# thomascbrs/mpc-tsid

Hardware: AMD Instinct MI355X
Metric: QP instances/s (12-state, N=16) at 1/2/4/8 MI355X; max |f - f_osqp| (higher is better)
Workload: dtype f64

## Files before the change

mpc-tsid_amd/csrc/mpcq_engine.hip:

```cpp
#include <math.h>

#include <type_traits>
#include <utility>

#include "mpcq_internal.h"

namespace mpcq {
namespace {

typedef __attribute__((address_space(3))) const double lds_cd;
typedef __attribute__((address_space(3))) double lds_d;
typedef double dbl2 __attribute__((ext_vector_type(2)));
typedef __attribute__((address_space(3))) const dbl2 lds_cd2;
typedef __attribute__((address_space(1))) const double g_cd;
typedef __attribute__((address_space(1))) double g_d;
typedef __attribute__((address_space(1))) const dbl2 g_cd2;

constexpr double kInf = 1e30;
constexpr double kMinScaling = 1e-4, kMaxScaling = 1e4;
constexpr double kRhoMin = 1e-6, kRhoMax = 1e6, kRhoEq = 1e3, kRhoTol = 1e-4;
constexpr double kDivTol = 1e-30;

enum : unsigned { RC_LOOSE = 0, RC_INEQ = 1, RC_EQ = 2 };

#if defined(MPCQ_STAMPS) && defined(MPCQ_STAMPS_LEAN)
#define STAMP_DECL uint64_t st_acc[16] = {}; uint64_t st_last = __builtin_amdgcn_s_memtime();
#define STAMP(i) do { if constexpr ((i) == 1 || (i) == 2 || (i) == 3 || (i) == 7 || (i) == 10 || (i) == 11 || (i) == 12) { \
    const uint64_t nw_ = __builtin_amdgcn_s_memtime(); st_acc[i] += nw_ - st_last; st_last = nw_; } } while (0)
#elif defined(MPCQ_STAMPS)
#define STAMP_DECL uint64_t st_acc[16] = {}; uint64_t st_last = __builtin_amdgcn_s_memtime();
#define STAMP(i) do { if (threadIdx.x == kStampT) { const uint64_t nw_ = __builtin_amdgcn_s_memtime(); st_acc[i] += nw_ - st_last; st_last = nw_; } } while (0)
#else
#define STAMP_DECL
#define STAMP(i) do {} while (0)
#endif

template <int N>
__device__ __forceinline__ int XO(int k, int i) {
  return (k < N - 1) ? 30 * k + (i < 6 ? 2 * i : 12 + 3 * (i - 6)) : 30 * (N - 1) + i;
}
template <int N>
__device__ __forceinline__ int FO(int k, int f, int c) {
  return 30 * N - 18 + 96 * k + 24 * f + 7 * c;
}
__host__ __device__ constexpr int LN(int psi) { return 4 * (psi / 3) + psi % 3; }

template <int N>
__host__ __device__ constexpr int SIG(int k) { return k <= N / 2 ? k : N + N / 2 - k; }
template <int N>
__host__ __device__ constexpr int SIGX(int q) { return q <= N / 2 ? q : N + N / 2 + 1 - q; }

template <int N>
constexpr int kRows = (N + 3) & ~3;
template <int N>
constexpr bool kSlice = slice_supported(N);


__device__ __forceinline__ void wave_sync() {
  __builtin_amdgcn_fence(__ATOMIC_RELEASE, "wavefront");
  __builtin_amdgcn_wave_barrier();
  asm volatile("" ::: "memory");
  __builtin_amdgcn_fence(__ATOMIC_ACQUIRE, "wavefront");
}
__device__ __forceinline__ void sync_all() { __syncthreads(); }

template <int CTRL>
__device__ __forceinline__ double dppd(double v) {
  return __longlong_as_double(__builtin_amdgcn_mov_dpp(__double_as_longlong(v), CTRL, 0xF, 0xF, false));
}
template <int J>
__device__ __forceinline__ double rbc(double v) { return dppd<0x150 + J>(v); }
template <int J>
__device__ __forceinline__ double qbc(double v) { return dppd<85 * J>(v); }
template <int J0, int J1, int J2, int J3>
__device__ __forceinline__ double qperm(double v) { return dppd<J0 + 4 * J1 + 16 * J2 + 64 * J3>(v); }

#define MPCQ_HV(i) "+v"(a[i])
#define MPCQ_HV4(i) MPCQ_HV(i), MPCQ_HV(i + 1), MPCQ_HV(i + 2), MPCQ_HV(i + 3)
template <int n>
__device__ __forceinline__ void hold_all(double (&a)[n]) {
  static_assert((n >= 1 && n <= 8) || n == 15 || n == 21, "hold_all: spell this count out");
  if constexpr (n == 1) asm volatile("" : MPCQ_HV(0));
  if constexpr (n == 2) asm volatile("" : MPCQ_HV(0), MPCQ_HV(1));
  if constexpr (n == 3) asm volatile("" : MPCQ_HV(0), MPCQ_HV(1), MPCQ_HV(2));
  if constexpr (n == 4) asm volatile("" : MPCQ_HV4(0));
  if constexpr (n == 5) asm volatile("" : MPCQ_HV4(0), MPCQ_HV(4));
  if constexpr (n == 6) asm volatile("" : MPCQ_HV4(0), MPCQ_HV(4), MPCQ_HV(5));
  if constexpr (n == 7) asm volatile("" : MPCQ_HV4(0), MPCQ_HV(4), MPCQ_HV(5), MPCQ_HV(6));
  if constexpr (n == 8) asm volatile("" : MPCQ_HV4(0), MPCQ_HV4(4));
  if constexpr (n == 15) asm volatile("" : MPCQ_HV4(0), MPCQ_HV4(4), MPCQ_HV4(8), MPCQ_HV(12), MPCQ_HV(13), MPCQ_HV(14));
  if constexpr (n == 21) asm volatile("" : MPCQ_HV4(0), MPCQ_HV4(4), MPCQ_HV4(8), MPCQ_HV4(12), MPCQ_HV4(16), MPCQ_HV(20));
}
#undef MPCQ_HV4
#undef MPCQ_HV

__device__ __forceinline__ double bdot12(const double (&g)[12], double v, double i0) {
  double a0 = i0;
  asm volatile("s_nop 1\n\t"
      "v_fmac_f64_dpp %0, %1, %2 row_newbcast:0 row_mask:0xf bank_mask:0xf\n\t"
      "v_fmac_f64_dpp %0, %1, %3 row_newbcast:1 row_mask:0xf bank_mask:0xf\n\t"
      "v_fmac_f64_dpp %0, %1, %4 row_newbcast:2 row_mask:0xf bank_mask:0xf\n\t"
      "v_fmac_f64_dpp %0, %1, %5 row_newbcast:3 row_mask:0xf bank_mask:0xf\n\t"
      "v_fmac_f64_dpp %0, %1, %6 row_newbcast:4 row_mask:0xf bank_mask:0xf\n\t"
      "v_fmac_f64_dpp %0, %1, %7 row_newbcast:5 row_mask:0xf bank_mask:0xf\n\t"
      "v_fmac_f64_dpp %0, %1, %8 row_newbcast:6 row_mask:0xf bank_mask:0xf\n\t"
      "v_fmac_f64_dpp %0, %1, %9 row_newbcast:7 row_mask:0xf bank_mask:0xf\n\t"
      "v_fmac_f64_dpp %0, %1, %10 row_newbcast:8 row_mask:0xf bank_mask:0xf\n\t"
      "v_fmac_f64_dpp %0, %1, %11 row_newbcast:9 row_mask:0xf bank_mask:0xf\n\t"
      "v_fmac_f64_dpp %0, %1, %12 row_newbcast:10 row_mask:0xf bank_mask:0xf\n\t"
      "v_fmac_f64_dpp %0, %1, %13 row_newbcast:11 row_mask:0xf bank_mask:0xf"
      : "+v"(a0)
      : "v"(v), "v"(g[0]), "v"(g[1]), "v"(g[2]), "v"(g[3]), "v"(g[4]), "v"(g[5]), "v"(g[6]), "v"(g[7]),
        "v"(g[8]), "v"(g[9]), "v"(g[10]), "v"(g[11]));
  return a0;
}
__device__ __forceinline__ double bdot_ln12(const double (&g)[12], double v, double i0) {
  double a0 = i0;
  asm("s_nop 1\n\t"
      "v_fmac_f64_dpp %0, %1, %2 row_newbcast:0 row_mask:0xf bank_mask:0xf\n\t"
      "v_fmac_f64_dpp %0, %1, %3 row_newbcast:1 row_mask:0xf bank_mask:0xf\n\t"
      "v_fmac_f64_dpp %0, %1, %4 row_newbcast:2 row_mask:0xf bank_mask:0xf\n\t"
      "v_fmac_f64_dpp %0, %1, %5 row_newbcast:4 row_mask:0xf bank_mask:0xf\n\t"
      "v_fmac_f64_dpp %0, %1, %6 row_newbcast:5 row_mask:0xf bank_mask:0xf\n\t"
      "v_fmac_f64_dpp %0, %1, %7 row_newbcast:6 row_mask:0xf bank_mask:0xf\n\t"
      "v_fmac_f64_dpp %0, %1, %8 row_newbcast:8 row_mask:0xf bank_mask:0xf\n\t"
      "v_fmac_f64_dpp %0, %1, %9 row_newbcast:9 row_mask:0xf bank_mask:0xf\n\t"
      "v_fmac_f64_dpp %0, %1, %10 row_newbcast:10 row_mask:0xf bank_mask:0xf\n\t"
      "v_fmac_f64_dpp %0, %1, %11 row_newbcast:12 row_mask:0xf bank_mask:0xf\n\t"
      "v_fmac_f64_dpp %0, %1, %12 row_newbcast:13 row_mask:0xf bank_mask:0xf\n\t"
      "v_fmac_f64_dpp %0, %1, %13 row_newbcast:14 row_mask:0xf bank_mask:0xf"
      : "+v"(a0)
      : "v"(v), "v"(g[0]), "v"(g[1]), "v"(g[2]), "v"(g[3]), "v"(g[4]), "v"(g[5]), "v"(g[6]), "v"(g[7]),
        "v"(g[8]), "v"(g[9]), "v"(g[10]), "v"(g[11]));
  return a0;
// ... 760 lines not shown
        return cl ? 0.0 : kInf;
      } else {
        return hi_g[j];
      }
    };

    using pdbl = __attribute__((address_space(5))) double;
    enum { ZC_LO = 0, ZC_HI = 3, ZC_RR = 6, ZC_RI = 9, ZC_COUNT = 12 };
    double zc_mem_[kZcMem<N> ? ZC_COUNT : 1];
    auto zc_ptr = [&]() __attribute__((always_inline)) -> pdbl* {
      pdbl* q = (pdbl*)&zc_mem_[0];
      asm volatile("" : "+v"(q));
      return q;
    };
    auto zc_store = [&]() __attribute__((always_inline)) {
      if constexpr (kZcMem<N>) {
        pdbl* const q = zc_ptr();
#pragma unroll
        for (int j = 0; j < 3; ++j) {
          q[ZC_LO + j] = lo_of(j);
          q[ZC_HI + j] = hi_of(j);
          q[ZC_RR + j] = rr[j];
          q[ZC_RI + j] = ri[j];
        }
      }
    };

    auto row_A = [&](double vf, double vX, double (&out)[3]) __attribute__((always_inline)) {
      double fall[12];
      gather12(vf, fall);
      const double* xp = sh.u.it.xs[k];
      const double hd = Hd(k, ph), h6 = H6(k, ph);
      const double xa = xp[ph], xb = xp[ph < 6 ? ph + 6 : ph];
      double dyn = Xd(k, ph) * vX;
      const double d1 = dyn + hd * xa;
      const double d2 = d1 + h6 * xb;
      dyn = k >= 1 ? (ph < 6 ? d2 : d1) : dyn;
      double bcf[12];
#pragma unroll
      for (int psi = 0; psi < 12; ++psi) bcf[psi] = Bc(k, ph, psi / 3, psi % 3);
      const double bf = dot12(bcf, fall);
      dyn = ph >= 6 ? dyn + bf : dyn;
      const double g0 = qbc<0>(vf), g1 = qbc<1>(vf), g2 = qbc<2>(vf);
      const double swg = Ab[fo + 4] * vf;
      out[0] = cl ? dyn : fric_row(3, g0, g1, g2);
      out[1] = cl ? swg : fric_row(4, g0, g1, g2);
      out[2] = cl ? fric_row(c, g0, g1, g2) : 0.0;
    };
    auto Pbf = [&]() __attribute__((always_inline)) { return cscale * (Df * P0f * Df); };
    auto PbX = [&]() __attribute__((always_inline)) { return cscale * (DX * P0X * DX); };

    auto rdy = [&](int kk, int i) __attribute__((always_inline)) { return GHr[GS * kk + 108 + i]; };
    auto Qv = [&](int kk, int j1, int j2) __attribute__((always_inline)) { return GHr[GS * kk + 6 * j1 + j2]; };
    auto Ctop = [&](int kk, int i, double& ca, double (&c6)[6]) __attribute__((always_inline)) {
      const int iq = i >= 6 ? i - 6 : 0;
      const double ri = rdy(kk, i), xi = Xd(kk, i), hi = Hd(kk, i), h6 = H6(kk, i < 6 ? i : 0);
      const double dv = ri * xi * hi, tv = ri * xi * h6;
      ca = i < 6 ? dv : 0.0;
#pragma unroll
      for (int j = 0; j < 6; ++j) {
        const double sc = xi * Qv(kk, iq, j) * Hd(kk, 6 + j);
        const double vv = (6 + j == i ? dv : 0.0) - sc;
        c6[j] = i < 6 ? (j == i ? tv : 0.0) : vv;
      }
    };
    auto Cbot = [&](int kk, int i, double& ca, double (&c6)[6]) __attribute__((always_inline)) {
      const int ip = i >= 6 ? i - 6 : 0;
      const double hi = Hd(kk, i);
      const double dv = rdy(kk, i) * Xd(kk, i) * hi;
      const double tv = rdy(kk, ip) * Xd(kk, ip) * H6(kk, ip);
      ca = i < 6 ? dv : tv;
#pragma unroll
      for (int j = 0; j < 6; ++j) {
        const double sc = Xd(kk, 6 + j) * Qv(kk, j, ip) * hi;
        const double vv = (6 + j == i ? dv : 0.0) - sc;
        c6[j] = i >= 6 ? vv : 0.0;
      }
    };
    auto Drow = [&](int kk, int i, double diag0, double (&Dr)[12]) __attribute__((always_inline)) {
      const bool nx = kk < N - 1;
      const int k1 = nx ? kk + 1 : kk;
      const int i6 = i < 6 ? i : i - 6, iq = i >= 6 ? i - 6 : 0;
      const double xi = Xd(kk, i), ri0 = rdy(kk, i);
      const double hi1 = Hd(k1, i), ri1 = rdy(k1, i);
      const double h6p = H6(k1, i6), rp1 = rdy(k1, i6), hp1 = Hd(k1, i6);
      double dg = diag0 + ri0 * xi * xi;
      const double dn = ri1 * hi1 * hi1 + (i >= 6 ? rp1 * h6p * h6p : 0.0);
      dg = nx ? dg + dn : dg;
      const double cross = nx ? (i < 6 ? ri1 * hi1 * h6p : rp1 * hp1 * h6p) : 0.0;
      const int partner = i < 6 ? i + 6 : i - 6;
#pragma unroll
      for (int ci = 0; ci < 12; ++ci) {
        double v = (ci == i) ? dg : 0.0;
        v = (ci == partner) ? cross : v;
        if (ci >= 6) {
          const double s0 = xi * Qv(kk, iq, ci - 6) * Xd(kk, ci);
          const double s1 = hi1 * Qv(k1, iq, ci - 6) * Hd(k1, ci);
          v = i >= 6 ? v - (nx ? s0 + s1 : s0) : v;
        }
        Dr[ci] = v;
      }
    };

      auto ph_sweep_lag = [&]() __attribute__((always_inline)) {
          const int half = (t >> 5) & 1;
#ifndef MPCQ_REP_SWEEP
#define MPCQ_REP_SWEEP 1
#endif
#pragma nounroll
          for (int rep_ = 0; rep_ < MPCQ_REP_SWEEP; ++rep_) {
          double xp = 0.0;
          using swp = lds_cd;
          using swp2 = lds_cd2;
          swp* const GHs = GHr;
          swp* const Mb = half == 0 ? GHs + (GS * (cr == 0 ? 0 : MID) + (cr == 0 ? 0 : kSlotPad<N>) + RS * rr_)
                                    : (swp*)&sh.Sm[0][0] + (GS * (cr == 0 ? -2 : MID - 1) + (cr == 0 ? 0 : kSlotPad<N>) + RS * rr_);
          double g[12];
          auto row12 = [&](swp* q) __attribute__((always_inline)) {
#pragma unroll
            for (int i = 0; i < 6; ++i) {
              const dbl2 v = ((swp2*)q)[i];
              g[2 * i] = v.x;
              g[2 * i + 1] = v.y;
            }
          };
          auto rowp = [&](int j) __attribute__((always_inline)) -> swp* {
            if (j >= 2 && j <= BOT) return Mb + GS * j;
            const int jj = half == 0 ? (cr == 0 ? j : (j < BOT ? j : BOT))
                                     : (cr == 0 ? (j > 2 ? j : 2) : (j < BOT + 1 ? j : BOT + 1));
            return Mb + GS * jj;
          };
          STAMP(15);
          if (t < 64) row12(rowp(1));
          sync_all();
          STAMP(3);
          lds_cd* const Ob = GHr + (GS * (cr == 0 ? 1 : N - MID) + (cr == 0 ? 0 : kSlotPad<N>) + rr_);
          if (t < 64) {
            __builtin_amdgcn_s_setprio(3);
            lds_cd* const Bb = (lds_cd*)&sh.u.it.bo[0][0] + (12 * (cr == 0 ? 0 : MID + 1) + rr_);
            lds_cd* const Bm = (lds_cd*)&sh.u.it.bo[0][0] + (12 * MID + rr_);
            auto rhs = [&](int j) __attribute__((always_inline)) -> lds_cd* {
              return (j >= BOT && cr != 0) ? Bm : Bb + 12 * j;
            };
            lds_d* const sink = (lds_d*)&sh.red[0] + (t & 31);
            lds_d* const Yb = (half == 1 && s < 12) ? (lds_d*)&sh.u.it.yv[0][0] + (12 * (cr == 0 ? -2 : MID - 1) + rr_)
                                                    : sink;
            lds_d* const Ym = ((N & 1) || cr == 0) ? Yb + 12 * (MID + 1) : sink;
            lds_d* const Pm = (half == 0 && cr == 0 && s < 12)
                                  ? (lds_d*)&sh.u.it.xs[0][0] + (12 * SIGX<N>(MID + 1) + rr_) : Ym;
            const double m0 = half == 0 ? 1.0 : 0.0;
// ... 30 lines not shown
              if (j >= 2 && j <= MID) {
                Yb[12 * j] = acc;
              } else if (j == MID + 1) {
                *Pm = acc;
              }
              if (j <= MID) {
                const bool adv = j <= BOT || cr == 0;
                src = keep_lo_take_lo(adv ? acc : src, src);
                asm volatile("" : "+v"(src));
              } else {
                xp = acc;
              }
            }
            STAMP(6);
          }
          if (t < 64) {
            lds_cd* const Wb = (lds_cd*)&sh.u.it.yv[0][0] + (12 * (cr == 0 ? 0 : N - MID) + rr_);
            lds_d* const sinkO = (lds_d*)&sh.red[0] + (t & 31);
            lds_d* const Xb = (half == 0 && s < 12) ? (lds_d*)&sh.u.it.xs[0][0] + (12 * (cr == 0 ? 1 : N - MID) + rr_)
                                                    : sinkO;
            wave_sync();
            double bq = Wb[12 * (MID - 1)];
#pragma unroll
            for (int j = 1; j <= MID; ++j) {
              asm volatile("" : : : "memory");
              double gc[12];
#pragma unroll
              for (int i = 0; i < 12; ++i) gc[i] = g[i];
              const double bc = bq;
              if (j < MID) {
#pragma unroll
                for (int i = 0; i < 12; ++i) g[i] = Ob[RS * i + GS * (MID - j - 1)];
                if (j + 1 <= BOT) bq = Wb[12 * (MID - j - 1)];
                else bq = Wb[12 * (MID - (cr == 0 ? j + 1 : BOT))];
              }
              asm volatile("" : : : "memory");
              const double acc = bdot12(gc, xp, bc);
              if (j < MID) {
                xp = acc;
                Xb[12 * (MID - j)] = acc;
              } else if constexpr (N & 1) {
                *Xb = acc;
              } else {
                *(cr == 0 ? Xb : sinkO) = acc;
              }
            }
            __builtin_amdgcn_s_setprio(0);
          }
          wave_sync();
          }
      };
    auto factor = [&](double sigma, const double* pr) __attribute__((always_inline)) -> bool {
      bool ok = true;
      launder();
      auto rho_of = [&](int j) __attribute__((always_inline)) -> double {
        return pr ? pr[j] : rho_of_cls(j);
      };
      double* gk = gh0 + GS * k;
      if (cl) gk[108 + ph] = rho_of(0);
      sync_all();
      {
        double rd6[6];
#pragma unroll
        for (int j = 0; j < 6; ++j) rd6[j] = gk[114 + j];
        double rfr[5];
        {
          const double r0 = rho_of(0), r1 = rho_of(1), r2 = rho_of(2);
          rfr[0] = qbc<0>(r2); rfr[1] = qbc<1>(r2); rfr[2] = qbc<2>(r2);
          rfr[3] = qbc<3>(r0); rfr[4] = qbc<3>(r1);
        }
        const double Bo0 = Ab[fo], Bo1 = Ab[fo + 1], Bo2 = Ab[fo + 2], Bo3 = Ab[fo + 3];
        const double sw = Ab[fo + 4];
        const double rsw = rho_of(1);
        double own_fr[5];
#pragma unroll
        for (int t_ = 0; t_ < 5; ++t_) own_fr[t_] = rfr[t_] * Frc(k, f, t_, cc);
        const double dgf = Pbf() + sigma + rsw * sw * sw;
#pragma unroll
        for (int psi = 0; psi < 12; ++psi) {
          const int fp = psi / 3, cp = psi % 3;
          double v = (cp == cc) ? rd6[cp] * Bo0 * Ab[FO<N>(k, fp, cp)] : 0.0;
          v += rd6[3] * Bo1 * Ab[FO<N>(k, fp, cp) + 1];
          v += rd6[4] * Bo2 * Ab[FO<N>(k, fp, cp) + 2];
          v += rd6[5] * Bo3 * Ab[FO<N>(k, fp, cp) + 3];
          if (psi == ph) v += dgf;
          if (fp == f) {
            double fr = 0.0;
#pragma unroll
            for (int t_ = 0; t_ < 5; ++t_) fr += own_fr[t_] * Frc(k, f, t_, cp);
            v += fr;
          }
          Fr[psi] = v;
        }
        gj12<!kBig<N>>(Fr, ph, ok);
        if constexpr (kFrWork<N>) {
#pragma unroll
          for (int i = 0; i < 12; ++i) FRg[16 * NR * i] = Fr[i];
        }
        double fw[6];
#pragma unroll
        for (int j = 0; j < 6; ++j) {
          double acc = 0.0;
#pragma unroll
          for (int psi = 0; psi < 12; ++psi) {
            const double bv = Bc(k, 6 + j, psi / 3, psi % 3);
            if (j >= 3 || psi % 3 == j) acc += Fr[psi] * (rd6[j] * bv);
          }
          fw[j] = acc;
        }
        if (cl) {
#pragma unroll
          for (int j = 0; j < 6; ++j) { gk[36 + 6 * ph + j] = fw[j]; FWW[kFWS<N> * k + 6 * ph + j] = fw[j]; }
        }
        wave_sync();
        for (int e = s; e < 36; e += 16) {
          const int j1 = e / 6, j2 = e % 6;
          const double r1 = gk[114 + j1];
          double acc = 0.0;
#pragma unroll
          for (int psi = 0; psi < 12; ++psi)
            acc += (r1 * Bc(k, 6 + j1, psi / 3, psi % 3)) * gk[36 + 6 * psi + j2];
          gk[e] = acc;
          QLW[36 * k + e] = acc / r1;
        }
      }
      const double dgX = PbX() + sigma;
      sync_all();
      STAMP(13);
      double* const St = sh.u.fa.St;
      double* const Sb = sh.u.fa.Sb;
      double Dr0[12], cta, ct6[6], cba, cb6[6];
      Drow(k, ph, dgX, Dr0);
      Ctop(k, ph, cta, ct6);
      Cbot(k < N - 1 ? k + 1 : k, ph, cba, cb6);
      auto couple = [&](bool upper, double (&Ro)[12]) __attribute__((always_inline)) {
        const double ca = upper ? cta : cba;
        double c6[6];
#pragma unroll
        for (int j = 0; j < 6; ++j) c6[j] = upper ? ct6[j] : cb6[j];
        const double* const Sp = upper ? St : Sb;
        wave_sync();
        const int ar = ph < 6 ? ph : ph - 6;
        double G[12];
        if constexpr (kBig<N>) {
#pragma unroll
          for (int ci = 0; ci < 12; ++ci) {
            double sv[7];
            sv[0] = Sp[12 * ar + ci];
#pragma unroll
            for (int j = 0; j < 6; ++j) sv[1 + j] = Sp[12 * (6 + j) + ci];
            double gv = ca * sv[0];
#pragma unroll
            for (int j = 0; j < 6; ++j) gv = fma(c6[j], sv[1 + j], gv);
            G[ci] = gv;
            asm volatile("" ::: "memory");
          }
        } else {
#pragma unroll
        for (int ci = 0; ci < 12; ci += 2) {
          const dbl2 s0 = *(lds_cd2*)(Sp + 12 * ar + ci);
          dbl2 su[6];
#pragma unroll
          for (int j = 0; j < 6; ++j) su[j] = *(lds_cd2*)(Sp + 12 * (6 + j) + ci);
          double g0 = ca * s0.x, g1 = ca * s0.y;
#pragma unroll
          for (int j = 0; j < 6; ++j) {
            g0 = fma(c6[j], su[j].x, g0);
            g1 = fma(c6[j], su[j].y, g1);
          }
          G[ci] = g0;
          G[ci + 1] = g1;
          asm volatile("" ::: "memory");
        }
        }
        if (cl) {
          double* const Gd = gh0 + SLOT<N>(upper ? SIG<N>(k) : SIG<N>(k + 1)) + RS * ph;
#pragma unroll
          for (int ci = 0; ci < 12; ++ci) Gd[ci] = -G[ci];
        }
        schur_cols<!kBig<N>>(Ro, G, ca, c6, std::make_integer_sequence<int, 12>{});
      };
#pragma nounroll
      for (int j = 0; j <= MID; ++j) {
        launder();
        const bool mid = j == MID;
        const bool top = !mid && k == j, bot = !mid && k == N - 1 - j && k > MID, mrow = mid && k == MID;
        if (top || bot || mrow) {
          const bool useT = (top && k > 0) || mrow, useB = (bot && k < N - 1) || mrow;
          double Ro[12];
#pragma unroll
          for (int ci = 0; ci < 12; ++ci) Ro[ci] = Dr0[ci];
          if (useT) couple(true, Ro);
          if (useB) couple(false, Ro);
          gj12<!kBig<N>>(Ro, ph, ok);
          if (cl) {
#pragma unroll
            for (int ci = 0; ci < 12; ++ci) SmW[SLOT<N>(SIG<N>(k)) + RS * ph + ci] = Ro[ci];
          }
          wave_sync();
          if (cl) {
            double* dst = mrow ? &sh.GH[0][RS * ph] : (bot ? Sb : St) + 12 * ph;
#pragma unroll
            for (int ci = 0; ci < 12; ++ci) dst[ci] = Ro[ci];
          }
        }
        sync_all();
      }
      STAMP(14);
      if (!ok) atomicOr(&sh.flag[2], 1);
      sync_all();
      const bool good = sh.flag[2] == 0;
      sync_all();
      return good;
    };

    double pri_res = 0.0, dua_res = 0.0, eps_pri = 0.0, eps_dua = 0.0, s_pri = 0.0, s_dua = 0.0;
    const bool hp = k >= 1, isv = ph >= 6;
    const int zXS = (int)(sh.zero - &sh.u.it.xs[0][0]);
    const double m2 = cc == 2 ? 1.0 : 0.0;
    int zAb;
    if constexpr (ABG) zAb = Work<N>::ZERO - Work<N>::AB;
    else zAb = (int)(sh.zero - sh.Ab);
    lds_cd* XSr = (lds_cd*)&sh.u.it.xs[0][0];
    double* const Wdump = &sh.dump[t & 63];
    struct LaneOffs {
      int oXd, oHd, oH6, oF, oFa, oFb, oF4, oFW, oQL, oXSp, oXSp6, rXS, rXSpm, rXSp6m, oHdm, oH6m, oFWcm, oQLm,
          oB0;
      bool ta0;
      double* Wbo;
      double* Wna;
    };
    auto offs = [&]() __attribute__((always_inline)) -> LaneOffs {
      const bool hp_ = k >= 1, isv_ = ph >= 6;
      LaneOffs o;
      o.oXd = xo;
      o.oHd = XO<N>(hp_ ? k - 1 : 0, ph) + (ph < 6 ? 1 : 2);
      o.oH6 = XO<N>(hp_ ? k - 1 : 0, ph < 6 ? ph + 6 : 11) + 1;
      o.oF = fo;
      const int ta = c < 3 ? c : 3;
      o.ta0 = (ta >> 1) == 0;
      o.oFa = FO<N>(k, f, ta >> 1) + 5 + (ta & 1);
      o.oFb = FO<N>(k, f, 2) + 5 + ta;
      o.oF4 = FO<N>(k, f, 2) + 9;
      o.oFW = kFWS<N> * k + 6 * ph;
      const int oFWc = kFWS<N> * k + (isv_ ? ph - 6 : 0);
      o.oQL = 36 * k + 6 * (isv_ ? ph - 6 : 0);
      o.oXSp = 12 * k + ph;
      o.oXSp6 = 12 * k + (ph < 6 ? ph + 6 : ph);
      auto xsl = [](int kk) __attribute__((always_inline)) -> int { return 12 * SIGX<N>(kk + 1); };
      o.rXS = xsl(k) + ph;
      o.rXSpm = hp_ ? xsl(k - 1) + ph : zXS;
      o.rXSp6m = hp_ ? xsl(k - 1) + (ph < 6 ? ph + 6 : ph) : zXS;
      o.oHdm = hp_ ? o.oHd : zAb;
      o.oH6m = hp_ && !isv_ ? o.oH6 : zAb;
      o.oFWcm = isv_ ? oFWc : zFW;
      o.oQLm = isv_ ? o.oQL : zQL;
      o.oB0 = FO<N>(k, 0, 0) + (ph >= 9 ? ph - 8 : 0);
      o.Wbo = &sh.u.it.bo[SIG<N>(k)][ph];
      o.Wna = &sh.u.it.na[SIG<N>(hp_ ? k - 1 : N - 1)][ph];
      return o;
    };
    LaneOffs O0 = offs();
#define MPCQ_LANE_OFFS(RECOMP)                                                                              \
  if constexpr (RECOMP) launder();                                                                         \
  const LaneOffs O_ = (RECOMP) ? offs() : O0;                                                              \
  [[maybe_unused]] const int oXd = O_.oXd, oHd = O_.oHd, oH6 = O_.oH6, oF = O_.oF, oFa = O_.oFa,           \
// ... 318 lines not shown
      eps_pri = p.eps_abs + p.eps_rel * fmax(qv[1], qv[2]);
      eps_dua = p.eps_abs + p.eps_rel * cinv * fmax(qv[7], qv[8]);
      s_pri = qv[3] / (fmax(qv[4], qv[5]) + kDivTol);
      s_dua = qv[9] / (fmax(qv[10], qv[11]) + kDivTol);
      pri_res = uni(pri_res); dua_res = uni(dua_res); eps_pri = uni(eps_pri);
      eps_dua = uni(eps_dua); s_pri = uni(s_pri); s_dua = uni(s_dua);

      if constexpr (INF) {
        const int e = s == 2 || s == 3 || s == 6 ? s : 0;
        double tv[NW];
#pragma unroll
        for (int w = 0; w < NW; ++w) tv[w] = D[DS * w + 16 + e];
        if constexpr (!BIG) hold_all(tv);
        double v = tv[0];
#pragma unroll
        for (int w = 1; w < NW; ++w) v = s == 6 ? v + tv[w] : fmax_hw(v, tv[w]);
        const double ndy = rbc<0>(v), ndx = rbc<2>(v), npdx = rbc<3>(v), ineq = rbc<6>(v);
        double epi0, edi0;
        chk_eps(epi0, edi0);
        int need = 0;
#pragma unroll
        for (int fi = 0; fi < 2; ++fi) {
          const double f = fi == 0 ? 1.0 : 10.0, epi = f * epi0, edi = f * edi0;
          const bool pi = !(pri_res < f * eps_pri) && ndy > kDivTol && ineq < epi * ndy;
          const bool di = !(dua_res < f * eps_dua) && ndx > kDivTol && 0.0 < csc * edi * ndx &&
                          npdx < csc * edi * ndx;
          need |= (pi ? 1 : 0) << (2 * fi);
          need |= (di ? 2 : 0) << (2 * fi);
        }
        inf_need = __builtin_amdgcn_readfirstlane(need);
        inf_bits = 0;
      }
    };
    auto update_info = [&](auto inf_tag, const double (&cv)[CK_COUNT]) __attribute__((always_inline)) {
      constexpr bool INF = decltype(inf_tag)::value;
      if constexpr (!INF) {
        if (cl) { sh.u.it.yv[k][ph] = xX; sh.u.it.bo[k][ph] = y[0]; }
        sync_all();
      }
      STAMP(4);
      launder_p();
      info_terms(cv, (lds_cd*)&sh.u.it.yv[0][0], &sh.u.it.bo[0][0], sh.red, 32);
      sync_all();
      STAMP(8);
      info_combine(inf_tag, cv, sh.red, 32);
      sync_all();
    };
    auto converged = [&](double fac) __attribute__((always_inline)) {
      return pri_res < fac * eps_pri && dua_res < fac * eps_dua;
    };

    if (status == 0) {
      STAMP(0);
      {
        double Pf = P0f, PX = P0X;
        double* Ex = gh0;
        auto fr_E = [&](int kk, int fp, int t_) __attribute__((always_inline)) {
          return t_ < 3 ? Ex[48 * kk + 3 * (4 * fp + t_) + 2] : Ex[48 * kk + 3 * (4 * fp + 3) + (t_ - 3)];
        };
        auto dyn_E = [&](int kk, int i) __attribute__((always_inline)) { return Ex[48 * kk + 3 * LN(i)]; };
        auto fr_norm = [&](int t_) __attribute__((always_inline)) {
          double v = fabs(Ab[FO<N>(k, f, 2) + 5 + t_]);
          if (t_ < 4) v = fmax(v, fabs(Ab[FO<N>(k, f, t_ >> 1) + 5 + (t_ & 1)]));
          return v;
        };
        for (int it = 0; it < p.scaling; ++it) {
          double dtf = fabs(Pf);
          {
            const int cnt = cc < 2 ? 7 : 10;
            for (int e = 0; e < cnt; ++e) dtf = fmax(dtf, fabs(Ab[fo + e]));
          }
          double dtx = fabs(PX);
          {
            const int cnt = (k < N - 1) ? (ph < 6 ? 2 : 3) : 1;
            for (int h = 0; h < cnt; ++h) dtx = fmax(dtx, fabs(Ab[xo + h]));
          }
          double et[3];
          {
            double v = fabs(Xd(k, ph));
            if (k >= 1) {
              v = fmax(v, fabs(Hd(k, ph)));
              if (ph < 6) v = fmax(v, fabs(H6(k, ph)));
            }
            if (ph >= 6) {
#pragma unroll
              for (int psi = 0; psi < 12; ++psi) v = fmax(v, fabs(Bc(k, ph, psi / 3, psi % 3)));
            }
            et[0] = cl ? v : fr_norm(3);
            et[1] = cl ? fabs(Ab[fo + 4]) : fr_norm(4);
            et[2] = cl ? fr_norm(c) : 0.0;
          }
          dtf = dtf < kMinScaling ? 1.0 : (dtf > kMaxScaling ? kMaxScaling : dtf);
          dtx = dtx < kMinScaling ? 1.0 : (dtx > kMaxScaling ? kMaxScaling : dtx);
          dtf = 1.0 / sqrt(dtf);
          dtx = 1.0 / sqrt(dtx);
          Df *= dtf;
          DX *= dtx;
          Pf = dtf * Pf * dtf;
          PX = dtx * PX * dtx;
#pragma unroll
          for (int j = 0; j < 3; ++j) {
            double v = et[j];
            v = v < kMinScaling ? 1.0 : (v > kMaxScaling ? kMaxScaling : v);
            et[j] = 1.0 / sqrt(v);
            E[j] *= et[j];
          }
#pragma unroll
          for (int j = 0; j < 3; ++j) Ex[48 * k + 3 * s + j] = et[j];
          sync_all();
          if (cl && !phantom) {
            const double dA = dyn_E(k, 6 + cc);
            AbW[fo] = dA * AbW[fo] * dtf;
#pragma unroll
            for (int j = 0; j < 3; ++j) AbW[fo + 1 + j] = dyn_E(k, 9 + j) * AbW[fo + 1 + j] * dtf;
            AbW[fo + 4] = et[1] * AbW[fo + 4] * dtf;
            if (cc < 2) {
              AbW[fo + 5] = fr_E(k, f, 2 * cc) * AbW[fo + 5] * dtf;
              AbW[fo + 6] = fr_E(k, f, 2 * cc + 1) * AbW[fo + 6] * dtf;
// ... 29 lines not shown
        }
      }
      if constexpr (FUSED) {
        bnd *= E[0];
      } else {
#pragma unroll
        for (int j = 0; j < 3; ++j) { lo_g[j] *= E[j]; hi_g[j] *= E[j]; }
      }
#pragma unroll
      for (int j = 0; j < 3; ++j) {
        const double lj = lo_of(j), hj = hi_of(j);
        unsigned cj;
        if (lj < -kInf * kMinScaling && hj > kInf * kMinScaling) cj = RC_LOOSE;
        else if (hj - lj < kRhoTol) cj = RC_EQ;
        else cj = RC_INEQ;
        cls |= cj << (2 * j);
      }
      set_rho();
      zc_store();
      if constexpr (!BIG) {
        pdbl* const q = ck_ptr();
        q[CK_DF] = Df; q[CK_DX] = DX; q[CK_PBF] = Pbf(); q[CK_PBX] = PbX(); q[CK_C] = cscale;
        q[CK_E0] = E[0]; q[CK_E1] = E[1]; q[CK_E2] = E[2]; q[CK_BND] = bnd;
      }
      if (a.warm_x && !first) {
        xf = a.warm_x[b * n + colF] / Df;
        xX = a.warm_x[b * n + colX] / DX;
        if (cl) sh.u.it.xs[k + 1][ph] = xX;
        sync_all();
        row_A(xf, xX, z);
        if (!cl) z[2] = 0.0;
        sync_all();
      }
      if (a.warm_y && !first) {
#pragma unroll
        for (int j = 0; j < 3; ++j) {
          const int r = nat_row(j);
          const double wy = r >= 0 ? a.warm_y[b * m + r] : 0.0;
          y[j] = r >= 0 ? (p.dual_warm ? wy : cscale * wy / E[j]) : 0.0;
        }
      }
      if constexpr (kSlice<N>) {
        if (a.resume) {
          constexpr int64_t RL = res_lanes(N);
          const double* const q = a.res + b * 8 * RL + t;
          xf = q[0];
          xX = q[RL];
#pragma unroll
          for (int j = 0; j < 3; ++j) { z[j] = q[(2 + j) * RL]; y[j] = q[(5 + j) * RL]; }
        }
      }
      sync_all();
      STAMP(1);

      constexpr bool kColfFold = !BIG;
      struct RhsOps {
        double cf[10], fwc[12], cXd, cHd, cH6;
        double cf0m[kColfFold ? 3 : 1];
      };
      auto load_rhs_ops = [&](RhsOps& o) __attribute__((always_inline)) {
        MPCQ_LANE_OFFS(true);
#pragma unroll
        for (int i = 0; i < 10; ++i) o.cf[i] = Ab[oF + i];
        if constexpr (kColfFold) {
          const int cs = cc == 0 ? 0 : (cc == 1 ? 1 : 2);
#pragma unroll
          for (int j = 0; j < 3; ++j) o.cf0m[j] = cs == j ? o.cf[0] : 0.0;
        }
#pragma unroll
        for (int psi = 0; psi < 12; ++psi) o.fwc[psi] = FWr[oFWcm + 6 * psi];
        o.cXd = Ab[oXd];
        o.cHd = Ab[oHdm];
        o.cH6 = Ab[oH6m];
      };
      auto ph_rhs = [&](bool admm, const RhsOps* op, const double (&pw)[3], double xcf, double xcX, double& uf,
                        double& beta) __attribute__((always_inline)) {
          if constexpr (kFrWork<N>) launder_p();
          RhsOps own_;
          if (!op) load_rhs_ops(own_);
          const RhsOps& o = op ? *op : own_;
          MPCQ_LANE_OFFS(kRecompLoop);
          double frg[12];
          if constexpr (kFrWork<N>) {
            g_cd* q = FRg;
            asm volatile("" : "+v"(q));
#pragma unroll
            for (int i = 0; i < 12; ++i) frg[i] = q[16 * NR * i];
          }
          const double cXd = o.cXd, cHd = o.cHd, cH6 = o.cH6;
          double w[3];
#pragma unroll
          for (int j = 0; j < 3; ++j) w[j] = admm ? rr[j] * z[j] - y[j] : pw[j];
          if constexpr (kZcMem<N>) {
            if (admm) {
              pdbl* const q = zc_ptr();
              const double r0 = q[ZC_RR], r1 = q[ZC_RR + 1], r2 = q[ZC_RR + 2];
              w[0] = r0 * z[0] - y[0];
              w[1] = r1 * z[1] - y[1];
              w[2] = r2 * z[2] - y[2];
            }
          }
          asm volatile("" : "+v"(w[0]), "+v"(w[1]), "+v"(w[2]) : : "memory");
          double colf;
          if constexpr (kColfFold) {
            double sA = -0.0, sB = -0.0;
            asm("s_nop 1\n\t"
// ... 566 lines not shown
              double cvq[CK_COUNT];
              ck_all(cvq);
              update_info(std::false_type{}, cvq);
            }
#ifdef MPCQ_DEBUG_POLISH
            if (b < 2 && t == 0) printf("blk %d rd %d admm pri %.3e dua %.3e | polished pri %.3e dua %.3e eps %.3e %.3e\n", (int)b, rd, a_pri, a_dua, pri_res, dua_res, eps_pri, eps_dua);
#endif
            if (!have || fmax(pri_res, dua_res) < fmax(b_pri, b_dua)) {
              have = true;
              b_pri = pri_res; b_dua = dua_res; b_epri = eps_pri; b_edua = eps_dua;
              bxf = xf; bxX = xX;
#pragma unroll
              for (int j = 0; j < 3; ++j) { bz[j] = z[j]; by[j] = y[j]; }
            }
          }
          const bool good = have && ((b_pri < a_pri && b_dua < a_dua) || (b_pri < a_pri && a_dua < 1e-10) ||
                                     (b_dua < a_dua && a_pri < 1e-10));
          if (good) {
            xf = bxf;
            xX = bxX;
#pragma unroll
            for (int j = 0; j < 3; ++j) { z[j] = bz[j]; y[j] = by[j]; }
            pol_st = 1;
            if (status != MPCQ_STATUS_SOLVED && b_pri < b_epri && b_dua < b_edua) status = MPCQ_STATUS_SOLVED;
          } else {
            xf = axf;
            xX = axX;
#pragma unroll
            for (int j = 0; j < 3; ++j) { z[j] = az[j]; y[j] = ay[j]; }
            pol_st = have ? -1 : 0;
          }
        }
      }
    }
    const bool nan_out = status == MPCQ_STATUS_NONFINITE || status == MPCQ_STATUS_FACTOR_FAILED ||
                         status == MPCQ_STATUS_BAD_GAIT || status == MPCQ_STATUS_BAD_BOUNDS ||
                         status == MPCQ_STATUS_PRIMAL_INFEASIBLE ||
                         status == MPCQ_STATUS_DUAL_INFEASIBLE || status == MPCQ_STATUS_PRIMAL_INFEASIBLE_INACCURATE ||
                         status == MPCQ_STATUS_DUAL_INFEASIBLE_INACCURATE;
    if (cl) {
      const double vf = nan_out ? NAN : Df * xf, vX = nan_out ? NAN : DX * xX;
      if (a.x) { a.x[b * n + colF] = vf; a.x[b * n + colX] = vX; }
      if (a.f0 && k == 0) a.f0[b * 12 + ph] = vf;
    }
    if (a.y) {
#pragma unroll
      for (int j = 0; j < 3; ++j) {
        const int r = nat_row(j);
        if (r >= 0) a.y[b * m + r] = nan_out ? NAN : (p.dual_warm ? y[j] : E[j] * y[j] / cscale);
      }
    }
#ifdef MPCQ_STAMPS
    STAMP(12);
    if (t == kStampT && a.stamps) {
      for (int i = 0; i < 16; ++i) a.stamps[b * 16 + i] = st_acc[i];
    }
#endif
    if (t == 0) {
      if (a.status) a.status[b] = status;
      if (a.iters) a.iters[b] = it_done;
      if (a.rho_out) a.rho_out[b] = rho_s;
      if (a.info) {
        a.info[4 * b + 0] = n_upd;
        a.info[4 * b + 1] = pol_st;
#ifdef MPCQ_FACTIME
        a.info[4 * b + 2] = (int)(fac_cycles >> 8);
#else
        a.info[4 * b + 2] = pol_rounds;
#endif
        a.info[4 * b + 3] = admm_st != 0 ? admm_st : status;
      }
    }
  }
}

template <int N>
hipError_t launch_t(bool fused, bool solve, const mpcq_params& p, const LaunchArgs& a,
                    hipStream_t s) {
  const dim3 grid((unsigned)a.batch), block(16 * kRows<N>);
  if (kBig<N> && solve && !a.work) return hipErrorInvalidValue;
  const bool pol = p.polish != 0;
  const bool rob = a.robots != nullptr && (fused || !solve);
  if (rob && solve && !a.weights) return hipErrorInvalidValue;
  if (!rob && a.weights) return hipErrorInvalidValue;
  if (rob && !solve) hipLaunchKernelGGL((engine_kernel<N, true, false, false, true>), grid, block, 0, s, p, a);
  else if (rob && pol) hipLaunchKernelGGL((engine_kernel<N, true, true, true, true>), grid, block, 0, s, p, a);
  else if (rob) hipLaunchKernelGGL((engine_kernel<N, true, true, false, true>), grid, block, 0, s, p, a);
  else if (!solve) hipLaunchKernelGGL((engine_kernel<N, true, false, false>), grid, block, 0, s, p, a);
  else if (fused && pol) hipLaunchKernelGGL((engine_kernel<N, true, true, true>), grid, block, 0, s, p, a);
  else if (fused) hipLaunchKernelGGL((engine_kernel<N, true, true, false>), grid, block, 0, s, p, a);
  else if (pol) hipLaunchKernelGGL((engine_kernel<N, false, true, true>), grid, block, 0, s, p, a);
  else hipLaunchKernelGGL((engine_kernel<N, false, true, false>), grid, block, 0, s, p, a);
  return hipGetLastError();
}

}

#ifndef MPCQ_ENGINE_N
#error "compile mpcq_engine.hip with -DMPCQ_ENGINE_N=<horizon> (see the Makefile)"
#endif
static_assert(MPCQ_ENGINE_N >= 4 && kRows<MPCQ_ENGINE_N> <= 64, "horizons 4..64 (1024 threads at most)");
static_assert(sizeof(Smem<MPCQ_ENGINE_N>) <= 160 * 1024, "Smem<N> exceeds the CU's LDS");
static_assert(!kBig<MPCQ_ENGINE_N> || Work<MPCQ_ENGINE_N>::SIZE == work_doubles(MPCQ_ENGINE_N),
              "work_doubles(N) (mpcq_internal.h) and Work<N> disagree");
static_assert(kRows<MPCQ_ENGINE_N> > 16 || sizeof(Smem<MPCQ_ENGINE_N>) <= 80 * 1024,
              "Smem<N> must fit twice in a CU for N <= 16");
// ... 10 lines not shown
```

Measured before the change: 137,900.

## Batch setup loads and vectorize factor stores for small-horizon path

For the non-BIG horizon, the Ruiz scaling loop is rewritten to gather all needed matrix entries into a 30-register array with branch-free zero-slot indexing, then apply updates. The factor routine builds the friction block with hoisted per-foot loads, reads X/H directly from the Ab matrix, writes Schur rows as 2-wide double stores with a wave-level sync, and drops two block barriers around the failure flag. It also adds optional setup timing stamps. The changes aim to cut scattered LDS loads and barriers in setup, at the cost of higher register pressure and more reliance on wave-level ordering.

New measurement: 137,500. No clear change (-0.3%).

```diff
diff --git a/mpc-tsid_amd/csrc/mpcq_engine.hip b/mpc-tsid_amd/csrc/mpcq_engine.hip
--- a/mpc-tsid_amd/csrc/mpcq_engine.hip
+++ b/mpc-tsid_amd/csrc/mpcq_engine.hip
@@ -34,6 +34,13 @@
 #define STAMP_DECL
 #define STAMP(i) do {} while (0)
 #endif
+#if defined(MPCQ_STAMPS) && defined(MPCQ_STAMPS_SETUP)
+#undef STAMP
+#define STAMP(i) do {} while (0)
+#define SSTAMP(i) do { if (threadIdx.x == kStampT) { const uint64_t nw_ = __builtin_amdgcn_s_memtime(); st_acc[i] += nw_ - st_last; st_last = nw_; } } while (0)
+#else
+#define SSTAMP(i) do {} while (0)
+#endif
 
 template <int N>
 __device__ __forceinline__ int XO(int k, int i) {
@@ -79,7 +86,12 @@
 #define MPCQ_HV4(i) MPCQ_HV(i), MPCQ_HV(i + 1), MPCQ_HV(i + 2), MPCQ_HV(i + 3)
 template <int n>
 __device__ __forceinline__ void hold_all(double (&a)[n]) {
-  static_assert((n >= 1 && n <= 8) || n == 15 || n == 21, "hold_all: spell this count out");
+  static_assert((n >= 1 && n <= 8) || n == 11 || n == 12 || n == 15 || n == 21 || n == 30,
+                "hold_all: spell this count out");
+  if constexpr (n == 11) asm volatile("" : MPCQ_HV4(0), MPCQ_HV4(4), MPCQ_HV(8), MPCQ_HV(9), MPCQ_HV(10));
+  if constexpr (n == 12) asm volatile("" : MPCQ_HV4(0), MPCQ_HV4(4), MPCQ_HV4(8));
+  if constexpr (n == 30) asm volatile("" : MPCQ_HV4(0), MPCQ_HV4(4), MPCQ_HV4(8), MPCQ_HV4(12), MPCQ_HV4(16), MPCQ_HV4(20),
+                                      MPCQ_HV4(24), MPCQ_HV(28), MPCQ_HV(29));
   if constexpr (n == 1) asm volatile("" : MPCQ_HV(0));
   if constexpr (n == 2) asm volatile("" : MPCQ_HV(0), MPCQ_HV(1));
   if constexpr (n == 3) asm volatile("" : MPCQ_HV(0), MPCQ_HV(1), MPCQ_HV(2));
@@ -946,27 +958,43 @@
 
     auto rdy = [&](int kk, int i) __attribute__((always_inline)) { return GHr[GS * kk + 108 + i]; };
     auto Qv = [&](int kk, int j1, int j2) __attribute__((always_inline)) { return GHr[GS * kk + 6 * j1 + j2]; };
+    auto XOb = [&](int kk, int i) __attribute__((always_inline)) -> int {
+      const int in = i + (i > 6 ? i - 6 : 0);
+      return 30 * kk + i + (int)(kk < N - 1) * in;
+    };
+    auto XdF = [&](int kk, int i) __attribute__((always_inline)) -> double {
+      if constexpr (kBig<N>) return Xd(kk, i);
+      else return Ab[XOb(kk, i)];
+    };
+    auto HdF = [&](int kk, int i) __attribute__((always_inline)) -> double {
+      if constexpr (kBig<N>) return Hd(kk, i);
+      else return Ab[XOb(kk > 0 ? kk - 1 : 0, i) + 1 + (int)(i >= 6)];
+    };
+    auto H6F = [&](int kk, int i) __attribute__((always_inline)) -> double {
+      if constexpr (kBig<N>) return H6(kk, i);
+      else return Ab[XOb(kk > 0 ? kk - 1 : 0, i < 6 ? i + 6 : 11) + 1];
+    };
     auto Ctop = [&](int kk, int i, double& ca, double (&c6)[6]) __attribute__((always_inline)) {
       const int iq = i >= 6 ? i - 6 : 0;
-      const double ri = rdy(kk, i), xi = Xd(kk, i), hi = Hd(kk, i), h6 = H6(kk, i < 6 ? i : 0);
+      const double ri = rdy(kk, i), xi = XdF(kk, i), hi = HdF(kk, i), h6 = H6F(kk, i < 6 ? i : 0);
       const double dv = ri * xi * hi, tv = ri * xi * h6;
       ca = i < 6 ? dv : 0.0;
 #pragma unroll
       for (int j = 0; j < 6; ++j) {
-        const double sc = xi * Qv(kk, iq, j) * Hd(kk, 6 + j);
+        const double sc = xi * Qv(kk, iq, j) * HdF(kk, 6 + j);
         const double vv = (6 + j == i ? dv : 0.0) - sc;
         c6[j] = i < 6 ? (j == i ? tv : 0.0) : vv;
       }
     };
     auto Cbot = [&](int kk, int i, double& ca, double (&c6)[6]) __attribute__((always_inline)) {
       const int ip = i >= 6 ? i - 6 : 0;
-      const double hi = Hd(kk, i);
-      const double dv = rdy(kk, i) * Xd(kk, i) * hi;
-      const double tv = rdy(kk, ip) * Xd(kk, ip) * H6(kk, ip);
+      const double hi = HdF(kk, i);
+      const double dv = rdy(kk, i) * XdF(kk, i) * hi;
+      const double tv = rdy(kk, ip) * XdF(kk, ip) * H6F(kk, ip);
       ca = i < 6 ? dv : tv;
 #pragma unroll
       for (int j = 0; j < 6; ++j) {
-        const double sc = Xd(kk, 6 + j) * Qv(kk, j, ip) * hi;
+        const double sc = XdF(kk, 6 + j) * Qv(kk, j, ip) * hi;
         const double vv = (6 + j == i ? dv : 0.0) - sc;
         c6[j] = i >= 6 ? vv : 0.0;
       }
@@ -975,9 +1003,9 @@
       const bool nx = kk < N - 1;
       const int k1 = nx ? kk + 1 : kk;
       const int i6 = i < 6 ? i : i - 6, iq = i >= 6 ? i - 6 : 0;
-      const double xi = Xd(kk, i), ri0 = rdy(kk, i);
-      const double hi1 = Hd(k1, i), ri1 = rdy(k1, i);
-      const double h6p = H6(k1, i6), rp1 = rdy(k1, i6), hp1 = Hd(k1, i6);
+      const double xi = XdF(kk, i), ri0 = rdy(kk, i);
+      const double hi1 = HdF(k1, i), ri1 = rdy(k1, i);
+      const double h6p = H6F(k1, i6), rp1 = rdy(k1, i6), hp1 = HdF(k1, i6);
       double dg = diag0 + ri0 * xi * xi;
       const double dn = ri1 * hi1 * hi1 + (i >= 6 ? rp1 * h6p * h6p : 0.0);
       dg = nx ? dg + dn : dg;
@@ -988,8 +1016,8 @@
         double v = (ci == i) ? dg : 0.0;
         v = (ci == partner) ? cross : v;
         if (ci >= 6) {
-          const double s0 = xi * Qv(kk, iq, ci - 6) * Xd(kk, ci);
-          const double s1 = hi1 * Qv(k1, iq, ci - 6) * Hd(k1, ci);
+          const double s0 = xi * Qv(kk, iq, ci - 6) * XdF(kk, ci);
+          const double s1 = hi1 * Qv(k1, iq, ci - 6) * HdF(k1, ci);
           v = i >= 6 ? v - (nx ? s0 + s1 : s0) : v;
         }
         Dr[ci] = v;
@@ -1126,6 +1154,7 @@
       };
     auto factor = [&](double sigma, const double* pr) __attribute__((always_inline)) -> bool {
       bool ok = true;
+      SSTAMP(15);
       launder();
       auto rho_of = [&](int j) __attribute__((always_inline)) -> double {
         return pr ? pr[j] : rho_of_cls(j);
@@ -1133,6 +1162,7 @@
       double* gk = gh0 + GS * k;
       if (cl) gk[108 + ph] = rho_of(0);
       sync_all();
+      SSTAMP(7);
       {
         double rd6[6];
 #pragma unroll
@@ -1150,6 +1180,39 @@
 #pragma unroll
         for (int t_ = 0; t_ < 5; ++t_) own_fr[t_] = rfr[t_] * Frc(k, f, t_, cc);
         const double dgf = Pbf() + sigma + rsw * sw * sw;
+        if constexpr (!kBig<N>) {
+          double frs[3];
+#pragma unroll
+          for (int cp = 0; cp < 3; ++cp) {
+            double fq[5];
+#pragma unroll
+            for (int t_ = 0; t_ < 5; ++t_) fq[t_] = Frc(k, f, t_, cp);
+            double fr = 0.0;
+#pragma unroll
+            for (int t_ = 0; t_ < 5; ++t_) fr += own_fr[t_] * fq[t_];
+            frs[cp] = fr;
+          }
+#pragma unroll
+          for (int fp = 0; fp < 4; ++fp) {
+            double av[12];
+#pragma unroll
+            for (int e = 0; e < 12; ++e) av[e] = Ab[FO<N>(k, fp, e >> 2) + (e & 3)];
+            hold_all(av);
+#pragma unroll
+            for (int cp = 0; cp < 3; ++cp) {
+              const int psi = 3 * fp + cp;
+              const double a0 = rd6[cp] * Bo0 * av[4 * cp];
+              double v = (cp == cc) ? a0 : 0.0;
+              v += rd6[3] * Bo1 * av[4 * cp + 1];
+              v += rd6[4] * Bo2 * av[4 * cp + 2];
+              v += rd6[5] * Bo3 * av[4 * cp + 3];
+              const double vd = v + dgf;
+              v = psi == ph ? vd : v;
+              const double vf = v + frs[cp];
+              Fr[psi] = fp == f ? vf : v;
+            }
+          }
+        } else {
 #pragma unroll
         for (int psi = 0; psi < 12; ++psi) {
           const int fp = psi / 3, cp = psi % 3;
@@ -1166,6 +1229,7 @@
           }
           Fr[psi] = v;
         }
+        }
         gj12<!kBig<N>>(Fr, ph, ok);
         if constexpr (kFrWork<N>) {
 #pragma unroll
@@ -1199,6 +1263,7 @@
         }
       }
       const double dgX = PbX() + sigma;
+      SSTAMP(8);
       sync_all();
       STAMP(13);
       double* const St = sh.u.fa.St;
@@ -1207,6 +1272,7 @@
       Drow(k, ph, dgX, Dr0);
       Ctop(k, ph, cta, ct6);
       Cbot(k < N - 1 ? k + 1 : k, ph, cba, cb6);
+      SSTAMP(9);
       auto couple = [&](bool upper, double (&Ro)[12]) __attribute__((always_inline)) {
         const double ca = upper ? cta : cba;
         double c6[6];
@@ -1249,8 +1315,13 @@
         }
         if (cl) {
           double* const Gd = gh0 + SLOT<N>(upper ? SIG<N>(k) : SIG<N>(k + 1)) + RS * ph;
-#pragma unroll
-          for (int ci = 0; ci < 12; ++ci) Gd[ci] = -G[ci];
+          if constexpr (kBig<N>) {
+#pragma unroll
+            for (int ci = 0; ci < 12; ++ci) Gd[ci] = -G[ci];
+          } else {
+#pragma unroll
+            for (int ci = 0; ci < 12; ci += 2) *(dbl2*)(Gd + ci) = dbl2{-G[ci], -G[ci + 1]};
+          }
         }
         schur_cols<!kBig<N>>(Ro, G, ca, c6, std::make_integer_sequence<int, 12>{});
       };
@@ -1264,9 +1335,13 @@
           double Ro[12];
 #pragma unroll
           for (int ci = 0; ci < 12; ++ci) Ro[ci] = Dr0[ci];
+          SSTAMP(13);
           if (useT) couple(true, Ro);
           if (useB) couple(false, Ro);
+          SSTAMP(10);
           gj12<!kBig<N>>(Ro, ph, ok);
+          SSTAMP(11);
+          if constexpr (kBig<N>) {
           if (cl) {
 #pragma unroll
             for (int ci = 0; ci < 12; ++ci) SmW[SLOT<N>(SIG<N>(k)) + RS * ph + ci] = Ro[ci];
@@ -1277,15 +1352,40 @@
 #pragma unroll
             for (int ci = 0; ci < 12; ++ci) dst[ci] = Ro[ci];
           }
+          } else {
+          if (cl) {
+            wdd* const sd = SmW + (SLOT<N>(SIG<N>(k)) + RS * ph);
+#pragma unroll
+            for (int ci = 0; ci < 12; ci += 2)
+              *(__attribute__((address_space(3))) dbl2*)(sd + ci) = dbl2{Ro[ci], Ro[ci + 1]};
+          }
+          wave_sync();
+          if (cl) {
+            double* dst = mrow ? &sh.GH[0][RS * ph] : (bot ? Sb : St) + 12 * ph;
+#pragma unroll
+            for (int ci = 0; ci < 12; ci += 2) *(dbl2*)(dst + ci) = dbl2{Ro[ci], Ro[ci + 1]};
+          }
+          }
+          SSTAMP(12);
+        }
+        if constexpr (!kBig<N>) {
+          if (mid && !ok) atomicOr(&sh.flag[2], 1);
         }
         sync_all();
       }
       STAMP(14);
+      SSTAMP(13);
+      if constexpr (!kBig<N>) {
+        const bool good = sh.flag[2] == 0;
+        SSTAMP(14);
+        return good;
+      } else {
       if (!ok) atomicOr(&sh.flag[2], 1);
       sync_all();
       const bool good = sh.flag[2] == 0;
       sync_all();
       return good;
+      }
     };
 
     double pri_res = 0.0, dua_res = 0.0, eps_pri = 0.0, eps_dua = 0.0, s_pri = 0.0, s_dua = 0.0;
@@ -1710,6 +1810,7 @@
 
     if (status == 0) {
       STAMP(0);
+      SSTAMP(0);
       {
         double Pf = P0f, PX = P0X;
         double* Ex = gh0;
@@ -1722,6 +1823,122 @@
           if (t_ < 4) v = fmax(v, fabs(Ab[FO<N>(k, f, t_ >> 1) + 5 + (t_ & 1)]));
           return v;
         };
+        if constexpr (!BIG) {
+          const int zA = (int)(sh.zero - sh.Ab);
+          const bool nx = k < N - 1;
+          const int k1 = nx ? k + 1 : k;
+          const int ta = cl ? c : 3;
+          const int iHd = XO<N>(k > 0 ? k - 1 : 0, ph) + (ph < 6 ? 1 : 2);
+          const int iH6 = XO<N>(k > 0 ? k - 1 : 0, ph < 6 ? ph + 6 : 11) + 1;
+          for (int it = 0; it < p.scaling; ++it) {
+            double L[30];
+            {
+              const int f7 = cc < 2 ? zA : fo;
+#pragma unroll
+              for (int e = 0; e < 10; ++e) L[e] = Ab[(e < 7 ? fo : f7) + e];
+              L[10] = Ab[xo];
+              L[11] = Ab[nx ? xo + 1 : zA];
+              L[12] = Ab[nx && ph >= 6 ? xo + 2 : zA];
+              L[13] = Ab[k >= 1 ? iHd : zA];
+              L[14] = Ab[k >= 1 && ph < 6 ? iH6 : zA];
+#pragma unroll
+              for (int psi = 0; psi < 12; ++psi) {
+                const int fp = psi / 3, cp = psi % 3;
+                const bool nz = ph >= 9 || (ph >= 6 && cp == ph - 6);
+                L[15 + psi] = Ab[nz ? FO<N>(k, fp, cp) + (ph >= 9 ? ph - 8 : 0) : zA];
+              }
+              L[27] = Ab[FO<N>(k, f, 2) + 5 + ta];
+              L[28] = Ab[FO<N>(k, f, ta >> 1) + 5 + (ta & 1)];
+              L[29] = Ab[FO<N>(k, f, 2) + 9];
+              hold_all(L);
+            }
+            double dtf = fabs(Pf);
+#pragma unroll
+            for (int e = 0; e < 10; ++e) dtf = fmax(dtf, fabs(L[e]));
+            double dtx = fabs(PX);
+#pragma unroll
+            for (int h = 0; h < 3; ++h) dtx = fmax(dtx, fabs(L[10 + h]));
+            double et[3];
+            {
+              double v = fabs(L[10]);
+              v = fmax(v, fabs(L[13]));
+              v = fmax(v, fabs(L[14]));
+#pragma unroll
+              for (int psi = 0; psi < 12; ++psi) v = fmax(v, fabs(L[15 + psi]));
+              const double fn = fmax(fabs(L[27]), fabs(L[28]));
+              et[0] = cl ? v : fn;
+              et[1] = cl ? fabs(L[4]) : fabs(L[29]);
+              et[2] = cl ? fn : 0.0;
+            }
+            dtf = dtf < kMinScaling ? 1.0 : (dtf > kMaxScaling ? kMaxScaling : dtf);
+            dtx = dtx < kMinScaling ? 1.0 : (dtx > kMaxScaling ? kMaxScaling : dtx);
+            dtf = 1.0 / sqrt(dtf);
+            dtx = 1.0 / sqrt(dtx);
+            Df *= dtf;
+            DX *= dtx;
+            Pf = dtf * Pf * dtf;
+            PX = dtx * PX * dtx;
+#pragma unroll
+            for (int j = 0; j < 3; ++j) {
+              double v = et[j];
+              v = v < kMinScaling ? 1.0 : (v > kMaxScaling ? kMaxScaling : v);
+              et[j] = 1.0 / sqrt(v);
+              E[j] *= et[j];
+            }
+#pragma unroll
+            for (int j = 0; j < 3; ++j) Ex[48 * k + 3 * s + j] = et[j];
+            SSTAMP(1);
+            sync_all();
+            SSTAMP(2);
+            if (cl && !phantom) {
+              double X[11];
+              X[0] = Ex[48 * k + 3 * LN(6 + cc)];
+#pragma unroll
+              for (int j = 0; j < 3; ++j) X[1 + j] = Ex[48 * k + 3 * LN(9 + j)];
+#pragma unroll
+              for (int j = 0; j < 5; ++j) {
+                const int tj = cc < 2 ? 2 * cc + (j & 1) : j;
+                X[4 + j] = Ex[48 * k + (tj < 3 ? 3 * (4 * f + tj) + 2 : 3 * (4 * f + 3) + (tj - 3))];
+              }
+              X[9] = Ex[48 * k1 + 3 * LN(ph >= 6 ? ph - 6 : ph)];
+              X[10] = Ex[48 * k1 + 3 * LN(ph)];
+              hold_all(X);
+              AbW[fo] = X[0] * L[0] * dtf;
+#pragma unroll
+              for (int j = 0; j < 3; ++j) AbW[fo + 1 + j] = X[1 + j] * L[1 + j] * dtf;
+              AbW[fo + 4] = et[1] * L[4] * dtf;
+              AbW[fo + 5] = X[4] * L[5] * dtf;
+              AbW[fo + 6] = X[5] * L[6] * dtf;
+              if (cc == 2) {
+#pragma unroll
+                for (int t_ = 2; t_ < 5; ++t_) AbW[fo + 5 + t_] = X[4 + t_] * L[5 + t_] * dtf;
+              }
+              AbW[xo] = et[0] * L[10] * dtx;
+              if (nx) {
+                AbW[xo + 1] = X[9] * L[11] * dtx;
+                if (ph >= 6) AbW[xo + 2] = X[10] * L[12] * dtx;
+              }
+            }
+            double ps = cl && !phantom ? fabs(Pf) + fabs(PX) : 0.0;
+            ps = wave_sum(ps);
+            double* const rp = sh.red + NW * (it & 1);
+            if ((t & 63) == 0) rp[wv] = ps;
+            SSTAMP(3);
+            sync_all();
+            SSTAMP(4);
+            ps = 0.0;
+#pragma unroll
+            for (int w = 0; w < NW; ++w) ps += rp[w];
+            const double mean = ps / n;
+            double ctmp = mean > 1.0 ? mean : 1.0;
+            ctmp = ctmp < kMinScaling ? 1.0 : (ctmp > kMaxScaling ? kMaxScaling : ctmp);
+            ctmp = 1.0 / ctmp;
+            Pf *= ctmp;
+            PX *= ctmp;
+            cscale = uni(cscale * ctmp);
+            SSTAMP(5);
+          }
+        } else
         for (int it = 0; it < p.scaling; ++it) {
           double dtf = fabs(Pf);
           {
@@ -1857,6 +2074,7 @@
       }
       sync_all();
       STAMP(1);
+      SSTAMP(6);
 
       constexpr bool kColfFold = !BIG;
       struct RhsOps {
@@ -2529,6 +2747,7 @@
     }
 #ifdef MPCQ_STAMPS
     STAMP(12);
+    SSTAMP(15);
     if (t == kStampT && a.stamps) {
       for (int i = 0; i < 16; ++i) a.stamps[b * 16 + i] = st_acc[i];
     }
```
